# kkrt-labs/stwo-brainfuck

Hardware: AMD Instinct MI355X
Metric: trace cells committed+proved/sec (higher is better)
Workload: dtype u32 (M31 / QM31 modular arithmetic)

## Files before the change

### stwo-brainfuck_amd/csrc/api.hip

```cpp
#include "../../include/bfhip.h"
#include "api_guard.h"
#include <cstdlib>
#include "host/circle.h"
#include "host/quotients.h"
#include "host/hash.h"
#include <cstdio>
#include <vector>
#include <algorithm>
#include <chrono>

using namespace bf;

static thread_local std::string g_err;
void bfhip_set_error(const std::string& s) { g_err = s; }

namespace bf {

void Ctx::ensure_aux() { for (auto& a : aux) if (!a) BF_HIP(hipStreamCreateWithFlags(&a, hipStreamNonBlocking)); }
void Ctx::ensure_side() { if (!stream2) BF_HIP(hipStreamCreateWithFlags(&stream2, hipStreamNonBlocking)); }

void Ctx::init(int dev, u32 max_log_domain, const Ctx* tables_from) {
    int n = 0;
    if (hipGetDeviceCount(&n) != hipSuccess || n == 0) throw HipError("no HIP device: the bfhip backend has no CPU fallback");
    if (dev < 0 || dev >= n) throw HipError("bad device id");
// ... 859 lines not shown
    for (int k = 0; k < N_COMPONENTS; k++) {
        claimed[k] = q_make(claimed_h[k].x, claimed_h[k].y, claimed_h[k].z, claimed_h[k].w);
        total = q_add(total, claimed[k]);
        reports[k] = check_report_init();
    }
    CheckLaunch launches[N_COMPONENTS];
    const CheckLaunch* d_launches = nullptr;
    CheckReportDev* d_reports = nullptr;
    {
        StageBatch sb(c);
        d_reports = c.stage(reports, N_COMPONENTS);
        for (int k = 0; k < N_COMPONENTS; k++) launches[k] = check_launch_of(k, log_sizes[k], rows[k], inter[k], el, claimed[k], d_reports + k);
        d_launches = c.stage(launches, N_COMPONENTS);
        sb.end();
    }
    {
        ProfScope ps(c.stream, "k_check_cells", 0);
        for (int k = 0; k < N_COMPONENTS; k++) check_constraints_launch(c.stream, k, d_launches + k, log_sizes[k]);
    }
    BF_HIP(hipGetLastError());
    c.read_back(reports, d_reports, sizeof reports);
    int32_t n_bad = 0;
    for (int k = 0; k < N_COMPONENTS; k++) { check_report_fill(out[k], reports[k], k, log_sizes[k], claimed[k]); n_bad += reports[k].n_bad_cells != 0; }
    logup_total_h[0] = total.a.a; logup_total_h[1] = total.a.b; logup_total_h[2] = total.b.a; logup_total_h[3] = total.b.b;
    if (n_bad_components) *n_bad_components = n_bad;
    return 0;
    API_CATCH
}
int32_t bfhip_accumulate_quotients(bfhip_ctx* ctx, uint32_t log_size, const uint32_t* const* cols_h, const uint32_t* col_shifts_h, uint32_t n_cols,
                                   const uint32_t* n_samples_h, const uint32_t* sample_points_h, const uint32_t* sample_values_h,
                                   const uint32_t random_coeff_h[4], uint32_t* const out_d[4]) {
    API_CTX(ctx)
    Ctx& c = ctx->c;
    if (log_size < 3 || log_size > c.tw_root_log + 1) throw HipError("accumulate_quotients: log_size outside the twiddle tree");
    std::vector<ColDesc> descs(n_cols);
    std::vector<std::vector<ColumnSample>> samples(n_cols);
    size_t si = 0;
    for (u32 k = 0; k < n_cols; k++) {
        descs[k] = ColDesc{cols_h[k], col_shifts_h ? col_shifts_h[k] : 0u, 0};
        if (descs[k].shift == 1) throw HipError("accumulate_quotients: column shift must be 0 or >= 2");
        for (u32 s = 0; s < n_samples_h[k]; s++, si++) {
            const uint32_t* p = sample_points_h + 8 * si;
            samples[k].push_back({PtQ{q_from_h(p), q_from_h(p + 4)}, q_from_h(sample_values_h + 4 * si)});
        }
    }
    std::vector<QuotientBatch> batches; std::vector<QuotientEntry> entries;
    build_quotient_batches(samples, q_from_h(random_coeff_h), batches, entries);
    quotient_entries_finish(batches.data(), batches.size(), entries.data(), descs.data());
    c.stage_checkpoint();
    QuotientArgs a{};
    a.batches = batches.empty() ? nullptr : c.stage(batches.data(), batches.size());
    a.entries = entries.empty() ? nullptr : c.stage(entries.data(), entries.size());
    a.n_batches = (u32)batches.size(); a.log = log_size; a.tw = c.d_tw; a.tw_total = 1u << c.tw_root_log;
    for (int w = 0; w < 4; w++) a.out[w] = out_d[w];
    const u32 blocks = quotient_groups_layout(&a, 1);
    accumulate_quotients(c.stream, c.stage(&a, 1), 1, blocks);
    BF_HIP(hipGetLastError());
    return 0;
    API_CATCH
}

}

#ifdef BFHIP_TEST_HOOKS
__global__ void __launch_bounds__(256) k_test_field_op(u32 op, const u32* __restrict__ a, const u32* __restrict__ b, u32* __restrict__ out, u32 n) {
    const u32 i = blockIdx.x * blockDim.x + threadIdx.x;
    if (i >= n) return;
    const u32 a0 = a[4 * i], a1 = a[4 * i + 1], a2 = a[4 * i + 2], a3 = a[4 * i + 3];
    const u32 b0 = b[4 * i], b1 = b[4 * i + 1], b2 = b[4 * i + 2], b3 = b[4 * i + 3];
    const u64 a64 = ((u64)a1 << 32) | a0;
    const Q31 x = q_make(a0, a1, a2, a3), y = q_make(b0, b1, b2, b3);
    Q31 r = q_zero();
    switch (op) {
        case 0: r.a.a = m_add(a0, b0); break;
        case 1: r.a.a = m_sub(a0, b0); break;
        case 2: r.a.a = m_mul(a0, b0); break;
        case 3: r.a.a = m_mul_pre2(a0, 2u * b0); break;
        case 4: r.a.a = m_mul_pow2(a0, b0 % 31u); break;
        case 5: r.a.a = m_inv(a0); break;
        case 6: r.a.a = m_red4(a64); break;
        case 7: r.a.a = m_canon(a64); break;
        case 8: r = q_mul(x, y); break;
        case 9: r = q_mul_const(x, q_const(y)); break;
        default: r = q_inv(x); break;
    }
    out[4 * i] = r.a.a; out[4 * i + 1] = r.a.b; out[4 * i + 2] = r.b.a; out[4 * i + 3] = r.b.b;
}
extern "C" int32_t bfhip_test_field_op(bfhip_ctx* ctx, uint32_t op, const uint32_t* a_d, const uint32_t* b_d, uint32_t* out_d, size_t n) {
    API_CTX(ctx)
    if (op > 10) throw HipError("bfhip_test_field_op: unknown op");
    if (!a_d || !b_d || !out_d) throw HipError("null argument");
    if (n == 0 || n > (size_t(1) << 28)) throw HipError("bfhip_test_field_op: n out of range");
    hipLaunchKernelGGL(k_test_field_op, dim3((u32)((n + 255) / 256)), dim3(256), 0, ctx->c.stream, op, a_d, b_d, out_d, (u32)n);
    BF_HIP(hipGetLastError());
    return 0;
    API_CATCH
}
extern "C" int32_t bfhip_test_constraint_group_rows(int32_t component, uint32_t log_size, uint32_t main_shift) {
    if (component < 0 || component >= N_COMPONENTS) { g_err = "unknown component"; return -1; }
    ConstraintLaunch L{};
    for (u32 j = 0; j < n_main_cols(component); j++) L.trace[j].shift = main_shift;
    for (u32 j = 0; j + 4 < 4 * n_logup_cols(component); j++) L.inter[j].shift = main_shift;
    L.log_size = log_size;
    return (int32_t)constraint_group_rows(L, component);
}
#endif
```

### stwo-brainfuck_amd/csrc/kernels.h

```cpp
#pragma once
#include <hip/hip_runtime.h>
#include "m31.h"
#include "air.h"
#include <string>
#include <vector>

struct bfhip_trace;

namespace bf {

struct ColDesc { const u32* ptr; u32 shift; u32 pad_; };

int prof_mode(hipStream_t s);
void prof_enable(hipStream_t s, int mode);
void prof_run_begin(hipStream_t s, const char* name);
void prof_run_end(hipStream_t s);
void prof_begin(hipStream_t s, const char* name, double bytes, double units, double aux = 0.0);
void prof_end(hipStream_t s);
void prof_reset(hipStream_t s);
std::string prof_report_json(const hipStream_t* streams, int n);
void prof_forget(hipStream_t s);
struct ProfScope {
    hipStream_t s; bool on;
    ProfScope(hipStream_t s_, const char* name, double bytes, double units = 0.0, bool dominant = false, double aux = 0.0) : s(s_) {
// ... 54 lines not shown
struct IsFirstCols { u32* ptr[28]; u32 log_min, log_max; };
void is_first_coeffs(hipStream_t stream, const IsFirstCols& a, const u32* itw, u32 tw_root_log);

void merkle_layer(hipStream_t stream, void* out, const void* prev, const ColDesc* d_cols, u32 ncols, u32 log, double col_bytes, u32 out_shift, u32 prev_shift,
                  u32 node_conv, u32 first = 0, u32 count = 0);
struct MerkleTreeDesc { uint4* layers[32]; u32 shifts[32]; u32 col_off[32]; const ColDesc* cols; u32 n_cols, max_log; };
static constexpr u32 MERKLE_SUBTREE_ROOT_LEVEL = 9;
void merkle_subtree(hipStream_t stream, const MerkleTreeDesc& tree, u32 hi, u32 node_conv, double bytes, double compressions);
void merkle_subtree_share(hipStream_t stream, const MerkleTreeDesc& tree, u32 hi, u32 stop, u32 lo, u32 wg0, u32 n_wg, u32 node_conv, double bytes, double compressions);
void merkle_top(hipStream_t stream, const MerkleTreeDesc& tree, u32 top_hi, u32 node_conv, u32* d_chan, u32* d_alpha8, u32* d_root_copy, double bytes, double compressions,
                u32* d_stamp = nullptr, u32 stamp_value = 0);
struct FriTailLayer {
    u32* ev[4];
    const u32* quot[4];
    uint4* tree[11];
};
struct FriTailArgs {
    u32 n_layers, top_log;
    u32 alpha_idx, root_idx;
    u32* ev_last[4];
    u32* chan; u32* alpha; u32* roots;
    const u32* itw; u32 tw_total, rfc;
    FriTailLayer layer[10];
};
void fri_tail(hipStream_t stream, const FriTailArgs* d_args, double bytes, double compressions);
struct FriLayerArgs {
    const u32* src[4]; const u32* quot[4]; u32* dst[4]; uint4* tree[18];
    const u32* alpha8; const u32* itw; u32 tw_total, log, rfc, pad_;
    u32* counter; u32* chan; u32* alpha_out; u32* root_out;
};
void fri_layer(hipStream_t stream, const FriLayerArgs& a);
enum FriFoldMode : int { FF_LINE = 0, FF_LINE_CIRCLE = 1, FF_CIRCLE = 2 };
struct FriFoldLeafArgs { const u32* src[4]; const u32* quot[4]; u32* dst[4]; const u32* alpha8; const u32* itw; u32 tw_total, log; };
void fri_fold_leaf(hipStream_t stream, void* out, const FriFoldLeafArgs& a, int mode, u32 node_conv);
void grind_span(hipStream_t stream, const u32* d_digest, u64 base, u32 span, u32 pow_bits, unsigned long long* d_best, u32 mix_u64_conv);
void clock_probe_launch(hipStream_t stream, uint4* d_stamps, u32* d_sink, u32 blocks, u32 iters);
void clock_sampler_launch(hipStream_t stream, uint4* d_out, const u32* d_stop_alias, unsigned long long max_ticks);
void fill_mix(hipStream_t stream, u32* p, size_t n);
void channel_mix_root_draw(hipStream_t stream, u32* d_chan, const u32* d_root, u32* d_alpha8, u32* d_root_copy);

void merkle_layer_poseidon(hipStream_t stream, void* out, const void* prev, const ColDesc* d_cols, u32 ncols, u32 log, u32 out_shift = 0, u32 prev_shift = 0,
                           u32 first = 0, u32 count = 0);
void hades_once(hipStream_t stream, const u32* d_in24, u32* d_out24);
void grind_poseidon_span(hipStream_t stream, const u32* d_digest, u64 base, u32 span, u32 pow_bits, unsigned long long* d_best);

struct ConstraintLaunch {
    const u32* is_first; ColDesc trace[13]; ColDesc inter[12]; u32* acc[4]; Q31 coeff[12]; Lookups el; Q31 total_sum; u32 denom_inv[2]; u32 log_size;
    u32 overwrite;
    u32 row0, n_rows;
    const u32* inter_prev[4];
};
void eval_constraints(hipStream_t stream, int comp, const ConstraintLaunch* d_args, u32 log_size, u32 n_rows = 0, u32 group_rows = 0);
u32 constraint_group_rows(const ConstraintLaunch& L, int comp);
struct ConstraintClass { u32 n_comps, block0, group_rows, pad_; u32 comp[13]; u32 pad2_[3]; };
struct ConstraintBatch { u32 n_classes, total_blocks, pad_[2]; ConstraintClass cls[13]; };
void constraint_batch_init(ConstraintBatch& b, const ConstraintLaunch* launches, u32 n);
void eval_constraints_batch(hipStream_t stream, const ConstraintBatch* d_batch, const ConstraintBatch& h_batch, const ConstraintLaunch* d_args);
struct LogupLaunch {
    const u32* cols[13];
    u32* out_rep[8];
    u32* out_last[4];
    void* vrow; void* wloc; void* totals; void* claimed;
    Lookups el; u32 log_rows; int comp;
};
struct LogupItem { const u32* cols[13]; u32* out_rep[8]; u32* out_last[4]; uint4* vrow; uint4* wloc; uint4* totals; uint4* claimed; u32 log_rows; int comp; u32 nb; u32 pad_; };
struct LogupBatch { Lookups el; u32 n; u32 rows_blk0[14], scan_blk0[14], last_blk0[14]; u32 pad_; LogupItem item[13]; };
void logup_batch_init(LogupBatch& b, const Lookups& el, const LogupLaunch* L, u32 n);
void logup_batch_run(hipStream_t stream, const LogupBatch* d_batch, const LogupBatch& h_batch);
void broadcast16(hipStream_t stream, const u32* d_rows, u32* d_out, u32 n_cells);

struct CheckReportDev { u64 n_bad_cells, first_bad_cell; u64 bad_per_constraint[16]; u32 first_bad_constraint; u32 first_bad_value[4]; u32 pad_[3]; };
struct CheckLaunch { ColDesc trace[13]; ColDesc inter[12]; Lookups el; Q31 total_sum; u32 log_size; u32 pad_; CheckReportDev* report; };
void check_constraints_launch(hipStream_t stream, int comp, const CheckLaunch* d_args, u32 log_size);

void trace_columns(const bfhip_trace* t, const u32* cols[N_COMPONENTS][13], u32 log_sizes[N_COMPONENTS]);

const u32* exclusive_scan_u32(hipStream_t s, const u32* in, u32* out, u32* totals, u32 n);

struct EvalJob { const u32* coeffs; u32 log_n; u32 point; u32 factor_shift; u32 partial_off; u32 out_idx; u32 pad_; };
void eval_at_points(hipStream_t stream, const EvalJob* d_jobs, u32 n_jobs, u32 total_partials, const void* d_factors, void* d_partials, void* d_out);
struct QuotientBatch { C31 prx, pry, pix, piy; Q31 a_sum, b_sum, batch_coeff; u32 n_cols; C31 kden; u32 n_full; };
struct QuotientEntry { Q31 c; const u32* ptr; u32 shift; u32 col; };
void quotient_entries_finish(QuotientBatch* batches, size_t n_batches, QuotientEntry* entries, const ColDesc* cols);
struct QuotientArgs { const QuotientBatch* batches; const QuotientEntry* entries; u32 n_batches; u32 log; const u32* tw; u32 tw_total; u32* out[4]; u32 row0, n_rows; u32 block0, pad_; };
u32 quotient_groups_layout(QuotientArgs* h_groups, u32 n_groups);
void accumulate_quotients(hipStream_t stream, const QuotientArgs* d_groups, u32 n_groups, u32 total_blocks);
void fold_circle_into_line(hipStream_t stream, u32* const dst[4], const u32* const src[4], const u32* d_alpha8, const u32* itw, u32 tw_root_log, u32 log, bool fresh = false,
                           u32 first = 0, u32 count = 0);
void fold_line(hipStream_t stream, u32* const dst[4], const u32* const src[4], const u32* d_alpha8, const u32* itw, u32 tw_root_log, u32 log, u32 first = 0, u32 count = 0);
void fold_line_circle(hipStream_t stream, u32* const dst[4], const u32* const src[4], const u32* const quot[4], const u32* d_alpha8, const u32* itw, u32 tw_root_log, u32 log,
                      u32 first = 0, u32 count = 0);
void prev_row_copy(hipStream_t stream, u32* dst, const u32* src, u32 log_size);
struct GatherReq { const u32* base; u64 index; u32 out_off; u32 n_words; };
void gather_u32(hipStream_t stream, const GatherReq* d_req, u32 n, u32* d_out);
void accumulate(hipStream_t stream, u32* dst, const u32* src, u32 n);
struct AccumulateSizes { u32* dst[4]; const u32* src[12][4]; u32 log[12]; u32 n; };
void accumulate_sizes(hipStream_t stream, const AccumulateSizes& a);
void batch_inverse_m31(hipStream_t stream, const u32* src, u32* dst, u32 n);
void batch_inverse_qm31(hipStream_t stream, const u32* const src[4], u32* const dst[4], u32 n);
void bit_reverse(hipStream_t stream, const u32* src, u32* dst, u32 log);
void one_hot(hipStream_t stream, u32* dst, u32 n);

struct TraceSoA { const u32 *clk, *ip, *ci, *ni, *mp, *mv, *mvi; u32 n; };
struct Ctx;
TraceSoA ingest_registers(Ctx& c, const u32* trace7_h, size_t n_rows, u64* first_bad);

}
```

### stwo-brainfuck_amd/csrc/m31.h

```cpp
#pragma once
#include <cstdint>
#include <cstddef>

#if defined(__HIPCC__)
#include <hip/hip_runtime.h>
#define BF_HD __host__ __device__ __forceinline__
#else
#define BF_HD inline
#endif

namespace bf {

using u8 = uint8_t;
using u32 = uint32_t;
using u64 = uint64_t;

constexpr u32 P31 = 0x7fffffffu;

struct Conventions {
    u32 merkle_node_hash = 0;
    u32 mix_u64 = 0;
    u32 logup_mask_order = 0;
    u32 merkle_channel = 0;
};

struct PcsConfig {
    u32 pow_bits = 5, log_blowup = 1, log_last_layer_degree_bound = 0, n_queries = 3;
    bool is_default() const { return pow_bits == 5 && log_blowup == 1 && log_last_layer_degree_bound == 0 && n_queries == 3; }
};

BF_HD u32 m_add(u32 a, u32 b) { u32 s = a + b; u32 t = s - P31; return t < s ? t : s; }
BF_HD u32 m_sub(u32 a, u32 b) { u32 s = a - b; u32 t = s + P31; return t < s ? t : s; }
BF_HD u64 m_fold(u64 x) { return (x & P31) + (x >> 31); }
BF_HD u32 m_canon(u64 x) { x = m_fold(m_fold(x)); u32 r = (u32)x; return r >= P31 ? r - P31 : r; }
BF_HD u32 m_neg(u32 a) { return a ? P31 - a : 0; }
BF_HD u32 m_reduce64(u64 x) {
    u32 lo = (u32)x & P31, hi = (u32)(x >> 31);
    u32 s = lo + hi; u32 t = s - P31; return t < s ? t : s;
}
BF_HD u32 m_mul(u32 a, u32 b) { return m_reduce64((u64)a * b); }
BF_HD u32 m_mul_pre2(u32 a, u32 w2) {
    u64 p = (u64)a * w2;
    u32 s = (u32)(p >> 32) + ((u32)p >> 1); u32 t = s - P31; return t < s ? t : s;
}
BF_HD u32 m_mul_pow2(u32 a, u32 k) { return ((a << k) & P31) | (a >> (31u - k)); }
BF_HD u32 m_sqr(u32 a) { return m_mul(a, a); }
BF_HD u32 m_inv_pow2(u32 n) { return 1u << ((31u - n % 31u) % 31u); }
BF_HD u32 m_pow(u32 b, u32 e) { u32 r = 1; while (e) { if (e & 1) r = m_mul(r, b); b = m_mul(b, b); e >>= 1; } return r; }
BF_HD u32 m_sqn(u32 x, int n) { for (int i = 0; i < n; i++) x = m_sqr(x); return x; }
BF_HD u32 m_inv(u32 x) {
    u32 t0 = m_mul(m_sqn(x, 2), x);
    u32 t1 = m_mul(m_sqr(t0), t0);
    u32 t2 = m_mul(m_sqn(t1, 3), t0);
    u32 t3 = m_mul(m_sqr(t2), t0);
    u32 t4 = m_mul(m_sqn(t3, 8), t3);
    u32 t5 = m_mul(m_sqn(t4, 8), t3);
    return m_mul(m_sqn(t5, 7), t2);
}

struct C31 { u32 a, b; };
BF_HD C31 c_add(C31 x, C31 y) { return {m_add(x.a, y.a), m_add(x.b, y.b)}; }
BF_HD C31 c_sub(C31 x, C31 y) { return {m_sub(x.a, y.a), m_sub(x.b, y.b)}; }
BF_HD C31 c_neg(C31 x) { return {m_neg(x.a), m_neg(x.b)}; }
BF_HD C31 c_mul(C31 x, C31 y) { return {m_sub(m_mul(x.a, y.a), m_mul(x.b, y.b)), m_add(m_mul(x.a, y.b), m_mul(x.b, y.a))}; }
BF_HD C31 c_mulm(C31 x, u32 y) { return {m_mul(x.a, y), m_mul(x.b, y)}; }
BF_HD C31 c_mulR(C31 x) { return {m_sub(m_add(x.a, x.a), x.b), m_add(x.a, m_add(x.b, x.b))}; }
BF_HD C31 c_inv(C31 x) { u32 n = m_inv(m_add(m_sqr(x.a), m_sqr(x.b))); return {m_mul(x.a, n), m_neg(m_mul(x.b, n))}; }

struct Q31 { C31 a, b; };
BF_HD Q31 q_make(u32 a0, u32 a1, u32 a2, u32 a3) { return {{a0, a1}, {a2, a3}}; }
BF_HD Q31 q_zero() { return {{0, 0}, {0, 0}}; }
BF_HD Q31 q_one() { return {{1, 0}, {0, 0}}; }
BF_HD Q31 q_from_m(u32 x) { return {{x, 0}, {0, 0}}; }
BF_HD Q31 q_add(Q31 x, Q31 y) { return {c_add(x.a, y.a), c_add(x.b, y.b)}; }
BF_HD Q31 q_sub(Q31 x, Q31 y) { return {c_sub(x.a, y.a), c_sub(x.b, y.b)}; }
BF_HD Q31 q_neg(Q31 x) { return {c_neg(x.a), c_neg(x.b)}; }
BF_HD Q31 q_mul(Q31 x, Q31 y) { return {c_add(c_mul(x.a, y.a), c_mulR(c_mul(x.b, y.b))), c_add(c_mul(x.a, y.b), c_mul(x.b, y.a))}; }
BF_HD Q31 q_mulm(Q31 x, u32 y) { return {c_mulm(x.a, y), c_mulm(x.b, y)}; }
struct QConst { u32 c0, c1, c2, c3, e0, e1, nc1, nc3, ne1; };
BF_HD QConst q_const(Q31 y) {
    const C31 e = c_mulR(y.b);
    return {y.a.a, y.a.b, y.b.a, y.b.b, e.a, e.b, P31 - y.a.b, P31 - y.b.b, P31 - e.b};
}
BF_HD u32 m_red4(u64 x) {
    const u64 t = ((x >> 32) << 1) + (u32)x;
    const u32 s = ((u32)t & P31) + (u32)(t >> 31); const u32 d = s - P31; return d < s ? d : s;
}
BF_HD Q31 q_mul_const(Q31 x, const QConst& k) {
    const u64 a0 = x.a.a, a1 = x.a.b, b0 = x.b.a, b1 = x.b.b;
    return q_make(m_red4(a0 * k.c0 + a1 * k.nc1 + b0 * k.e0 + b1 * k.ne1), m_red4(a0 * k.c1 + a1 * k.c0 + b0 * k.e1 + b1 * k.e0),
                  m_red4(a0 * k.c2 + a1 * k.nc3 + b0 * k.c0 + b1 * k.nc1), m_red4(a0 * k.c3 + a1 * k.c2 + b0 * k.c1 + b1 * k.c0));
}
BF_HD Q31 q_mulc(Q31 x, C31 y) { return {c_mul(x.a, y), c_mul(x.b, y)}; }
BF_HD Q31 q_addm(Q31 x, u32 y) { x.a.a = m_add(x.a.a, y); return x; }
BF_HD Q31 q_subm(Q31 x, u32 y) { x.a.a = m_sub(x.a.a, y); return x; }
BF_HD Q31 q_conj(Q31 x) { return {x.a, c_neg(x.b)}; }
BF_HD Q31 q_inv(Q31 x) { C31 d = c_inv(c_sub(c_mul(x.a, x.a), c_mulR(c_mul(x.b, x.b)))); return {c_mul(x.a, d), c_neg(c_mul(x.b, d))}; }
BF_HD bool q_eq(Q31 x, Q31 y) { return x.a.a == y.a.a && x.a.b == y.a.b && x.b.a == y.b.a && x.b.b == y.b.b; }
BF_HD bool q_is_zero(Q31 x) { return (x.a.a | x.a.b | x.b.a | x.b.b) == 0; }
BF_HD Q31 q_pow(Q31 b, u64 e) { Q31 r = q_one(); while (e) { if (e & 1) r = q_mul(r, b); b = q_mul(b, b); e >>= 1; } return r; }

BF_HD u32 bit_rev(u32 i, u32 log) {
#if defined(__HIP_DEVICE_COMPILE__)
    return log ? (__brev(i) >> (32 - log)) : 0;
#else
    u32 r = 0; for (u32 k = 0; k < log; k++) r |= ((i >> k) & 1u) << (log - 1 - k); return r;
#endif
}

}
```

### stwo-brainfuck_amd/csrc/quotient.hip

```cpp
#include <algorithm>
#include "kernels.h"
#include <stdexcept>

namespace bf {

__device__ __forceinline__ Q31 ld_q(const uint4* p, size_t i) { uint4 v = p[i]; return q_make(v.x, v.y, v.z, v.w); }
__device__ __forceinline__ uint4 pk_q(Q31 q) { return make_uint4(q.a.a, q.a.b, q.b.a, q.b.b); }

static constexpr u32 EAP_CHUNK_LOG = 12;

__global__ void __launch_bounds__(256) k_eval_at_point_stage1(const EvalJob* __restrict__ jobs, u32 n_jobs, const uint4* __restrict__ factors, uint4* __restrict__ partials) {
    u32 lo_j = 0, hi_j = n_jobs;
    while (hi_j - lo_j > 1) { u32 mid = (lo_j + hi_j) >> 1; if (jobs[mid].partial_off <= blockIdx.x) lo_j = mid; else hi_j = mid; }
    const EvalJob job = jobs[lo_j];
    const u32 n = 1u << job.log_n;
    const u32 chunk = blockIdx.x - job.partial_off;
    __shared__ uint4 s_w[16];
    __shared__ uint4 s_p[256];
    const uint4* F = factors + (size_t)job.point * 32 + job.factor_shift;
    const u32 t = threadIdx.x;
    if (t < 16) {
        Q31 w = q_one();
        for (u32 b = 0; b < 4; b++) if ((t >> b) & 1) w = q_mul(w, ld_q(F, b));
        s_w[t] = pk_q(w);
// ... 8 lines not shown
#pragma unroll
            for (u32 v4 = 0; v4 < 4; v4++) {
                const uint4 c = src[v4];
                const u32 cv[4] = {c.x, c.y, c.z, c.w};
#pragma unroll
                for (u32 j = 0; j < 4; j++) {
                    const u32 idx = v4 * 4 + j;
                    if (idx % 4 == 0 && idx) { a64[0] = m_fold(a64[0]); a64[1] = m_fold(a64[1]); a64[2] = m_fold(a64[2]); a64[3] = m_fold(a64[3]); }
                    const Q31 w = ld_q(s_w, idx);
                    a64[0] += (u64)w.a.a * cv[j]; a64[1] += (u64)w.a.b * cv[j]; a64[2] += (u64)w.b.a * cv[j]; a64[3] += (u64)w.b.b * cv[j];
                }
            }
            acc = q_make(m_red4(a64[0]), m_red4(a64[1]), m_red4(a64[2]), m_red4(a64[3]));
        } else {
            for (u32 k = 0; k < n; k++) acc = q_add(acc, q_mulm(ld_q(s_w, k), job.coeffs[k]));
        }
    }
    s_p[t] = pk_q(acc);
    __syncthreads();
    for (u32 b = 0; b < 8; b++) {
        u32 half = 128u >> b;
        Q31 r;
        bool act = t < half;
        if (act) {
            Q31 lo = ld_q(s_p, 2 * t), hi = ld_q(s_p, 2 * t + 1);
            r = (4 + b < job.log_n) ? q_add(lo, q_mul_const(hi, q_const(ld_q(F, 4 + b)))) : lo;
        }
        __syncthreads();
        if (act) s_p[t] = pk_q(r);
        __syncthreads();
    }
    if (t == 0) partials[(size_t)job.partial_off + chunk] = s_p[0];
}

__global__ void __launch_bounds__(256) k_eval_at_point_stage2(const EvalJob* __restrict__ jobs, const uint4* __restrict__ factors, const uint4* __restrict__ partials, uint4* __restrict__ out) {
    const EvalJob job = jobs[blockIdx.x];
    const u32 nchunks = job.log_n > EAP_CHUNK_LOG ? 1u << (job.log_n - EAP_CHUNK_LOG) : 1u;
    const uint4* F = factors + (size_t)job.point * 32 + job.factor_shift;
    const uint4* p = partials + job.partial_off;
    __shared__ uint4 s[256];
    const u32 t = threadIdx.x;
    u32 lanes = nchunks < 256 ? nchunks : 256;
    u32 per_log = 0; while ((lanes << per_log) < nchunks) per_log++;
    Q31 acc = q_zero();
    if (t < lanes) {
        u32 per = 1u << per_log;
        for (u32 k = 0; k < per; k++) {
            Q31 w = q_one();
            for (u32 b = 0; b < per_log; b++) if ((k >> b) & 1) w = q_mul(w, ld_q(F, EAP_CHUNK_LOG + b));
            acc = q_add(acc, q_mul(ld_q(p, ((size_t)t << per_log) + k), w));
        }
    }
    s[t] = pk_q(acc);
    __syncthreads();
    u32 lanes_log = 0; while ((1u << lanes_log) < lanes) lanes_log++;
    for (u32 b = 0; b < lanes_log; b++) {
        u32 half = lanes >> (b + 1);
        Q31 r; bool act = t < half;
        if (act) r = q_add(ld_q(s, 2 * t), q_mul_const(ld_q(s, 2 * t + 1), q_const(ld_q(F, EAP_CHUNK_LOG + per_log + b))));
        __syncthreads();
        if (act) s[t] = pk_q(r);
        __syncthreads();
    }
    if (t == 0) out[job.out_idx] = s[0];
}

void eval_at_points(hipStream_t stream, const EvalJob* d_jobs, u32 n_jobs, u32 total_partials, const void* d_factors, void* d_partials, void* d_out) {
    if (!n_jobs) return;
    hipLaunchKernelGGL(k_eval_at_point_stage1, dim3(total_partials), dim3(256), 0, stream, d_jobs, n_jobs, (const uint4*)d_factors, (uint4*)d_partials);
    hipLaunchKernelGGL(k_eval_at_point_stage2, dim3(n_jobs), dim3(256), 0, stream, d_jobs, (const uint4*)d_factors, (const uint4*)d_partials, (uint4*)d_out);
}

__device__ __forceinline__ void domain_point(const u32* __restrict__ tw, u32 tw_total, u32 log, u32 row, u32& x, u32& y) {
    const u32* t1 = tw + (tw_total - (1u << (log - 1)));
    u32 xv = t1[row >> 2];
    x = (row & 2) ? m_neg(xv) : xv;
    u32 h = row >> 1;
    u32 cx = t1[(h >> 2) * 2], cy = t1[(h >> 2) * 2 + 1];
    u32 sel = h & 3;
    u32 yv = sel == 0 ? cy : sel == 1 ? m_neg(cy) : sel == 2 ? m_neg(cx) : cx;
    y = (row & 1) ? m_neg(yv) : yv;
}

__global__ void __launch_bounds__(256) k_quotients(const QuotientArgs* __restrict__ groups, u32 n_groups) {
    u32 g = 0;
    while (g + 1 < n_groups && groups[g + 1].block0 <= blockIdx.x) g++;
    const QuotientArgs& a = groups[g];
    u32 row0 = ((blockIdx.x - a.block0) * blockDim.x + threadIdx.x) * 4;
    if (a.n_rows) { if (row0 >= a.n_rows) return; row0 += a.row0; }
    else if (row0 >= (1u << a.log)) return;
    u32 xv, yv;
    domain_point(a.tw, a.tw_total, a.log, row0, xv, yv);
    Q31 acc[4] = {q_zero(), q_zero(), q_zero(), q_zero()};
    u32 e = 0;
    for (u32 b = 0; b < a.n_batches; b++) {
        const QuotientBatch qb = ld_constant(a.batches + b);
        u64 n64[4][4], s64[4];
#pragma unroll
        for (int r = 0; r < 4; r++) { n64[r][0] = 0; n64[r][1] = 0; n64[r][2] = 0; n64[r][3] = 0; }
        s64[0] = 0; s64[1] = 0; s64[2] = 0; s64[3] = 0;
        const QuotientEntry* ent = a.entries + e;
        e += qb.n_cols;
        const u32 nf = qb.n_full, nr = qb.n_cols - qb.n_full;
        if (nf) {
            uint4 A[3], B[3];
            const u32 last = nf - 1;
            auto load3 = [&](uint4 (&buf)[3], u32 k) {
#pragma unroll
                for (u32 j = 0; j < 3; j++) buf[j] = ld16(as_global(ld_constant(&ent[min(k + j, last)].ptr)) + row0);
            };
            auto mac3 = [&](const uint4 (&buf)[3], u32 k) {
#pragma unroll
                for (int r = 0; r < 4; r++) { n64[r][0] = m_fold(n64[r][0]); n64[r][1] = m_fold(n64[r][1]); n64[r][2] = m_fold(n64[r][2]); n64[r][3] = m_fold(n64[r][3]); }
#pragma unroll
                for (u32 j = 0; j < 3; j++) {
                    if (k + j < nf) {
                        const Q31 cc = ld_constant(&ent[k + j].c);
                        const u32 vr[4] = {buf[j].x, buf[j].y, buf[j].z, buf[j].w};
#pragma unroll
                        for (int r = 0; r < 4; r++) { n64[r][0] += (u64)cc.a.a * vr[r]; n64[r][1] += (u64)cc.a.b * vr[r]; n64[r][2] += (u64)cc.b.a * vr[r]; n64[r][3] += (u64)cc.b.b * vr[r]; }
                    }
                }
            };
            load3(A, 0);
            for (u32 k = 0; k < nf; k += 6) {
                load3(B, k + 3);
                mac3(A, k);
                load3(A, k + 6);
                mac3(B, k + 3);
            }
        }
        if (nr) {
            const QuotientEntry* er = ent + nf;
            u32 A[3], B[3];
            const u32 last = nr - 1;
            auto load3 = [&](u32 (&buf)[3], u32 k) {
#pragma unroll
                for (u32 j = 0; j < 3; j++) { const u32 i = min(k + j, last); buf[j] = as_global(ld_constant(&er[i].ptr))[row0 >> ld_constant(&er[i].shift)]; }
            };
            auto mac3 = [&](const u32 (&buf)[3], u32 k) {
                s64[0] = m_fold(s64[0]); s64[1] = m_fold(s64[1]); s64[2] = m_fold(s64[2]); s64[3] = m_fold(s64[3]);
#pragma unroll
                for (u32 j = 0; j < 3; j++) {
                    if (k + j < nr) {
                        const Q31 cc = ld_constant(&er[k + j].c);
                        s64[0] += (u64)cc.a.a * buf[j]; s64[1] += (u64)cc.a.b * buf[j]; s64[2] += (u64)cc.b.a * buf[j]; s64[3] += (u64)cc.b.b * buf[j];
                    }
                }
            };
            load3(A, 0);
            for (u32 k = 0; k < nr; k += 6) {
                load3(B, k + 3);
                mac3(A, k);
                load3(A, k + 6);
                mac3(B, k + 3);
            }
        }
        const Q31 ay = q_mulm(qb.a_sum, yv);
        const Q31 line_p = q_add(qb.b_sum, ay), line_m = q_sub(qb.b_sum, ay);
        const C31 P = {m_mul(xv, qb.piy.a), m_mul(xv, qb.piy.b)}, Q = {m_mul(yv, qb.pix.a), m_mul(yv, qb.pix.b)};
        const C31 km = c_sub(qb.kden, P), kp = c_add(qb.kden, P);
        C31 den[4] = {c_add(km, Q), c_sub(km, Q), c_sub(kp, Q), c_add(kp, Q)};
        Q31 num[4]; u32 nrm[4];
#pragma unroll
        for (int r = 0; r < 4; r++) {
            num[r] = q_make(m_canon(m_fold(n64[r][0]) + m_fold(s64[0])), m_canon(m_fold(n64[r][1]) + m_fold(s64[1])),
                            m_canon(m_fold(n64[r][2]) + m_fold(s64[2])), m_canon(m_fold(n64[r][3]) + m_fold(s64[3])));
            num[r] = q_sub(num[r], (r == 0 || r == 3) ? line_p : line_m);
            nrm[r] = m_add(m_sqr(den[r].a), m_sqr(den[r].b));
        }
        u32 p01 = m_mul(nrm[0], nrm[1]), p012 = m_mul(p01, nrm[2]), inv_all = m_inv(m_mul(p012, nrm[3]));
        u32 i3 = m_mul(inv_all, p012), t3 = m_mul(inv_all, nrm[3]);
        u32 i2 = m_mul(t3, p01), t2 = m_mul(t3, nrm[2]);
        u32 i1 = m_mul(t2, nrm[0]), i0 = m_mul(t2, nrm[1]);
        u32 ninv[4] = {i0, i1, i2, i3};
#pragma unroll
        for (int r = 0; r < 4; r++) {
            C31 dinv = {m_mul(den[r].a, ninv[r]), m_neg(m_mul(den[r].b, ninv[r]))};
            Q31 term = q_mulc(num[r], dinv);
            acc[r] = b ? q_add(acc[r], term) : term;
        }
    }
    *reinterpret_cast<uint4*>(a.out[0] + row0) = make_uint4(acc[0].a.a, acc[1].a.a, acc[2].a.a, acc[3].a.a);
    *reinterpret_cast<uint4*>(a.out[1] + row0) = make_uint4(acc[0].a.b, acc[1].a.b, acc[2].a.b, acc[3].a.b);
    *reinterpret_cast<uint4*>(a.out[2] + row0) = make_uint4(acc[0].b.a, acc[1].b.a, acc[2].b.a, acc[3].b.a);
    *reinterpret_cast<uint4*>(a.out[3] + row0) = make_uint4(acc[0].b.b, acc[1].b.b, acc[2].b.b, acc[3].b.b);
}
void quotient_entries_finish(QuotientBatch* batches, size_t n_batches, QuotientEntry* entries, const ColDesc* cols) {
    for (size_t b = 0; b < n_batches; b++) {
        QuotientEntry* first = entries; QuotientEntry* last = entries + batches[b].n_cols;
        for (QuotientEntry* q = first; q != last; q++) { q->ptr = cols[q->col].ptr; q->shift = cols[q->col].shift; }
        batches[b].n_full = (u32)(std::stable_partition(first, last, [](const QuotientEntry& q) { return q.shift == 0; }) - first);
        entries = last;
    }
}
u32 quotient_groups_layout(QuotientArgs* h_groups, u32 n_groups) {
    u32 blocks = 0;
    for (u32 g = 0; g < n_groups; g++) {
        const u32 lanes = (h_groups[g].n_rows ? h_groups[g].n_rows : (1u << h_groups[g].log)) / 4;
        h_groups[g].block0 = blocks;
        blocks += (lanes + 255) / 256;
    }
    return blocks;
}
void accumulate_quotients(hipStream_t stream, const QuotientArgs* d_groups, u32 n_groups, u32 total_blocks) {
    if (!n_groups || !total_blocks) return;
    ProfScope ps(stream, "k_quotients", 0);
    hipLaunchKernelGGL(k_quotients, dim3(total_blocks), dim3(256), 0, stream, d_groups, n_groups);
}

__global__ void __launch_bounds__(256) k_fold_circle_into_line(u32* const d0, u32* const d1, u32* const d2, u32* const d3,
                                                               const u32* __restrict__ s0, const u32* __restrict__ s1, const u32* __restrict__ s2, const u32* __restrict__ s3,
                                                               const u32* __restrict__ alpha8, const u32* __restrict__ itw, u32 tw_total, u32 log, u32 fresh, u32 first, u32 count) {
    u32 i = blockIdx.x * blockDim.x + threadIdx.x;
    if (i >= count) return;
    i += first;
    const QConst alpha = q_const(q_make(alpha8[0], alpha8[1], alpha8[2], alpha8[3])), alpha_sq = q_const(q_make(alpha8[4], alpha8[5], alpha8[6], alpha8[7]));
    const u32* t1 = itw + (tw_total - (1u << (log - 1)));
    u32 cx = t1[(i >> 2) * 2], cy = t1[(i >> 2) * 2 + 1], sel = i & 3;
    u32 yinv = sel == 0 ? cy : sel == 1 ? m_neg(cy) : sel == 2 ? m_neg(cx) : cx;
    uint2 a0 = reinterpret_cast<const uint2*>(s0)[i], a1 = reinterpret_cast<const uint2*>(s1)[i], a2 = reinterpret_cast<const uint2*>(s2)[i], a3 = reinterpret_cast<const uint2*>(s3)[i];
    Q31 fp = q_make(a0.x, a1.x, a2.x, a3.x), fn = q_make(a0.y, a1.y, a2.y, a3.y);
    Q31 f0 = q_add(fp, fn), f1 = q_mulm(q_sub(fp, fn), yinv);
    Q31 fprime = q_add(q_mul_const(f1, alpha), f0);
    Q31 r = fprime;
    if (!fresh) { Q31 dst = q_make(d0[i], d1[i], d2[i], d3[i]); r = q_add(q_mul_const(dst, alpha_sq), fprime); }
    d0[i] = r.a.a; d1[i] = r.a.b; d2[i] = r.b.a; d3[i] = r.b.b;
}
__global__ void __launch_bounds__(256) k_fold_line(u32* __restrict__ d0, u32* __restrict__ d1, u32* __restrict__ d2, u32* __restrict__ d3,
                                                   const u32* __restrict__ s0, const u32* __restrict__ s1, const u32* __restrict__ s2, const u32* __restrict__ s3,
                                                   const u32* __restrict__ alpha8, const u32* __restrict__ itw, u32 tw_total, u32 log, u32 first, u32 count) {
    u32 i = blockIdx.x * blockDim.x + threadIdx.x;
    if (i >= count) return;
    i += first;
    const QConst alpha = q_const(q_make(alpha8[0], alpha8[1], alpha8[2], alpha8[3]));
    u32 xinv = itw[tw_total - (1u << log) + i];
    uint2 a0 = reinterpret_cast<const uint2*>(s0)[i], a1 = reinterpret_cast<const uint2*>(s1)[i], a2 = reinterpret_cast<const uint2*>(s2)[i], a3 = reinterpret_cast<const uint2*>(s3)[i];
    Q31 fx = q_make(a0.x, a1.x, a2.x, a3.x), fn = q_make(a0.y, a1.y, a2.y, a3.y);
    Q31 f0 = q_add(fx, fn), f1 = q_mulm(q_sub(fx, fn), xinv);
    Q31 r = q_add(f0, q_mul_const(f1, alpha));
    d0[i] = r.a.a; d1[i] = r.a.b; d2[i] = r.b.a; d3[i] = r.b.b;
}
__global__ void __launch_bounds__(256) k_fold_line_circle(u32* __restrict__ d0, u32* __restrict__ d1, u32* __restrict__ d2, u32* __restrict__ d3,
                                                          const u32* __restrict__ s0, const u32* __restrict__ s1, const u32* __restrict__ s2, const u32* __restrict__ s3,
                                                          const u32* __restrict__ q0, const u32* __restrict__ q1, const u32* __restrict__ q2, const u32* __restrict__ q3,
                                                          const u32* __restrict__ alpha8, const u32* __restrict__ itw, u32 tw_total, u32 log, u32 first, u32 count) {
    u32 i = blockIdx.x * blockDim.x + threadIdx.x;
    if (i >= count) return;
    i += first;
    const QConst alpha = q_const(q_make(alpha8[0], alpha8[1], alpha8[2], alpha8[3]));
    Q31 r;
    {
        const u32 xinv = itw[tw_total - (1u << log) + i];
        const uint2 a0 = reinterpret_cast<const uint2*>(s0)[i], a1 = reinterpret_cast<const uint2*>(s1)[i], a2 = reinterpret_cast<const uint2*>(s2)[i], a3 = reinterpret_cast<const uint2*>(s3)[i];
        const Q31 fx = q_make(a0.x, a1.x, a2.x, a3.x), fn = q_make(a0.y, a1.y, a2.y, a3.y);
        r = q_add(q_add(fx, fn), q_mul_const(q_mulm(q_sub(fx, fn), xinv), alpha));
    }
    if (q0) {
        const QConst alpha_sq = q_const(q_make(alpha8[4], alpha8[5], alpha8[6], alpha8[7]));
        const u32* t1 = itw + (tw_total - (1u << (log - 1)));
        const u32 cx = t1[(i >> 2) * 2], cy = t1[(i >> 2) * 2 + 1], sel = i & 3;
        const u32 yinv = sel == 0 ? cy : sel == 1 ? m_neg(cy) : sel == 2 ? m_neg(cx) : cx;
        const uint2 a0 = reinterpret_cast<const uint2*>(q0)[i], a1 = reinterpret_cast<const uint2*>(q1)[i], a2 = reinterpret_cast<const uint2*>(q2)[i], a3 = reinterpret_cast<const uint2*>(q3)[i];
        const Q31 fp = q_make(a0.x, a1.x, a2.x, a3.x), fn = q_make(a0.y, a1.y, a2.y, a3.y);
        const Q31 fprime = q_add(q_mul_const(q_mulm(q_sub(fp, fn), yinv), alpha), q_add(fp, fn));
        r = q_add(q_mul_const(r, alpha_sq), fprime);
    }
    d0[i] = r.a.a; d1[i] = r.a.b; d2[i] = r.b.a; d3[i] = r.b.b;
}
void fold_line_circle(hipStream_t stream, u32* const dst[4], const u32* const src[4], const u32* const quot[4], const u32* d_alpha8, const u32* itw, u32 tw_root_log, u32 log,
                      u32 first, u32 count) {
    if (!count) { first = 0; count = 1u << (log - 1); }
    hipLaunchKernelGGL(k_fold_line_circle, dim3((count + 255) / 256), dim3(256), 0, stream, dst[0], dst[1], dst[2], dst[3], src[0], src[1], src[2], src[3],
                       quot ? quot[0] : nullptr, quot ? quot[1] : nullptr, quot ? quot[2] : nullptr, quot ? quot[3] : nullptr, d_alpha8, itw, 1u << tw_root_log, log, first, count);
}

void fold_circle_into_line(hipStream_t stream, u32* const dst[4], const u32* const src[4], const u32* d_alpha8, const u32* itw, u32 tw_root_log, u32 log, bool fresh,
                           u32 first, u32 count) {
    if (!count) { first = 0; count = 1u << (log - 1); }
    hipLaunchKernelGGL(k_fold_circle_into_line, dim3((count + 255) / 256), dim3(256), 0, stream, dst[0], dst[1], dst[2], dst[3], src[0], src[1], src[2], src[3],
                       d_alpha8, itw, 1u << tw_root_log, log, fresh ? 1u : 0u, first, count);
}
// ... 101 lines not shown
```

Before: 14.37 billion.

## Batch quotient denominator inversions across four batches and widen single-batch lanes

Restructures the quotient kernel so each lane computes denominators for up to four batches (or four quads of rows in the single-batch case), stores them in shared memory, and shares one field inversion across all of them (Montgomery batch inversion). When a group has a single batch, each lane handles 16 rows and writes terms directly, so one inversion covers sixteen rows. The column loads use a deeper 4-entry prefetch pipeline, and a lazy complex multiply skips some reductions. This trades inversion cost for 32KB of shared memory per block, which may reduce occupancy, and for added code complexity.

```diff
diff --git a/stwo-brainfuck_amd/csrc/api.hip b/stwo-brainfuck_amd/csrc/api.hip
--- a/stwo-brainfuck_amd/csrc/api.hip
+++ b/stwo-brainfuck_amd/csrc/api.hip
@@ -965,19 +965,27 @@
         case 7: r.a.a = m_canon(a64); break;
         case 8: r = q_mul(x, y); break;
         case 9: r = q_mul_const(x, q_const(y)); break;
-        default: r = q_inv(x); break;
+        case 10: r = q_inv(x); break;
+        case 11: r.a.a = c_norm(x.a); break;
+        default: r = q_mulc_lazy(x, y.a); break;
     }
     out[4 * i] = r.a.a; out[4 * i + 1] = r.a.b; out[4 * i + 2] = r.b.a; out[4 * i + 3] = r.b.b;
 }
 extern "C" int32_t bfhip_test_field_op(bfhip_ctx* ctx, uint32_t op, const uint32_t* a_d, const uint32_t* b_d, uint32_t* out_d, size_t n) {
     API_CTX(ctx)
-    if (op > 10) throw HipError("bfhip_test_field_op: unknown op");
+    if (op > 12) throw HipError("bfhip_test_field_op: unknown op");
     if (!a_d || !b_d || !out_d) throw HipError("null argument");
     if (n == 0 || n > (size_t(1) << 28)) throw HipError("bfhip_test_field_op: n out of range");
     hipLaunchKernelGGL(k_test_field_op, dim3((u32)((n + 255) / 256)), dim3(256), 0, ctx->c.stream, op, a_d, b_d, out_d, (u32)n);
     BF_HIP(hipGetLastError());
     return 0;
     API_CATCH
+}
+extern "C" int32_t bfhip_test_quotient_rows_per_lane(uint32_t log_size, uint32_t n_rows, uint32_t n_batches) {
+    QuotientArgs a{};
+    a.log = log_size; a.n_rows = n_rows; a.n_batches = n_batches;
+    quotient_groups_layout(&a, 1);
+    return (int32_t)a.rows_per_lane;
 }
 extern "C" int32_t bfhip_test_constraint_group_rows(int32_t component, uint32_t log_size, uint32_t main_shift) {
     if (component < 0 || component >= N_COMPONENTS) { g_err = "unknown component"; return -1; }
diff --git a/stwo-brainfuck_amd/csrc/kernels.h b/stwo-brainfuck_amd/csrc/kernels.h
--- a/stwo-brainfuck_amd/csrc/kernels.h
+++ b/stwo-brainfuck_amd/csrc/kernels.h
@@ -160,7 +160,7 @@
 struct QuotientBatch { C31 prx, pry, pix, piy; Q31 a_sum, b_sum, batch_coeff; u32 n_cols; C31 kden; u32 n_full; };
 struct QuotientEntry { Q31 c; const u32* ptr; u32 shift; u32 col; };
 void quotient_entries_finish(QuotientBatch* batches, size_t n_batches, QuotientEntry* entries, const ColDesc* cols);
-struct QuotientArgs { const QuotientBatch* batches; const QuotientEntry* entries; u32 n_batches; u32 log; const u32* tw; u32 tw_total; u32* out[4]; u32 row0, n_rows; u32 block0, pad_; };
+struct QuotientArgs { const QuotientBatch* batches; const QuotientEntry* entries; u32 n_batches; u32 log; const u32* tw; u32 tw_total; u32* out[4]; u32 row0, n_rows; u32 block0, rows_per_lane; };
 u32 quotient_groups_layout(QuotientArgs* h_groups, u32 n_groups);
 void accumulate_quotients(hipStream_t stream, const QuotientArgs* d_groups, u32 n_groups, u32 total_blocks);
 void fold_circle_into_line(hipStream_t stream, u32* const dst[4], const u32* const src[4], const u32* d_alpha8, const u32* itw, u32 tw_root_log, u32 log, bool fresh = false,
diff --git a/stwo-brainfuck_amd/csrc/m31.h b/stwo-brainfuck_amd/csrc/m31.h
--- a/stwo-brainfuck_amd/csrc/m31.h
+++ b/stwo-brainfuck_amd/csrc/m31.h
@@ -92,6 +92,12 @@
                   m_red4(a0 * k.c2 + a1 * k.nc3 + b0 * k.c0 + b1 * k.nc1), m_red4(a0 * k.c3 + a1 * k.c2 + b0 * k.c1 + b1 * k.c0));
 }
 BF_HD Q31 q_mulc(Q31 x, C31 y) { return {c_mul(x.a, y), c_mul(x.b, y)}; }
+BF_HD u32 c_norm(C31 x) { return m_red4((u64)x.a * x.a + (u64)x.b * x.b); }
+BF_HD C31 c_mul_lazy(C31 x, C31 y) {
+    const u32 nb = P31 - y.b;
+    return {m_red4((u64)x.a * y.a + (u64)x.b * nb), m_red4((u64)x.a * y.b + (u64)x.b * y.a)};
+}
+BF_HD Q31 q_mulc_lazy(Q31 x, C31 y) { return {c_mul_lazy(x.a, y), c_mul_lazy(x.b, y)}; }
 BF_HD Q31 q_addm(Q31 x, u32 y) { x.a.a = m_add(x.a.a, y); return x; }
 BF_HD Q31 q_subm(Q31 x, u32 y) { x.a.a = m_sub(x.a.a, y); return x; }
 BF_HD Q31 q_conj(Q31 x) { return {x.a, c_neg(x.b)}; }
diff --git a/stwo-brainfuck_amd/csrc/quotient.hip b/stwo-brainfuck_amd/csrc/quotient.hip
--- a/stwo-brainfuck_amd/csrc/quotient.hip
+++ b/stwo-brainfuck_amd/csrc/quotient.hip
@@ -114,109 +114,164 @@
     y = (row & 1) ? m_neg(yv) : yv;
 }
 
+
+__device__ __forceinline__ void quad_dens(const QuotientBatch& qb, u32 xv, u32 yv, C31 (&den)[4]) {
+    const C31 P = {m_mul(xv, qb.piy.a), m_mul(xv, qb.piy.b)}, Q = {m_mul(yv, qb.pix.a), m_mul(yv, qb.pix.b)};
+    const C31 km = c_sub(qb.kden, P), kp = c_add(qb.kden, P);
+    den[0] = c_add(km, Q); den[1] = c_sub(km, Q); den[2] = c_sub(kp, Q); den[3] = c_add(kp, Q);
+}
+
+template <bool SETTLE> __device__ __forceinline__ void quad_numerators(const QuotientEntry* ent, u32 nf, u32 nr, u32 row0, Q31 (&num)[4]) {
+    u64 n64[4][4], s64[4];
+#pragma unroll
+    for (int r = 0; r < 4; r++) { n64[r][0] = 0; n64[r][1] = 0; n64[r][2] = 0; n64[r][3] = 0; }
+    s64[0] = 0; s64[1] = 0; s64[2] = 0; s64[3] = 0;
+    if (nf) {
+        uint4 buf[4];
+        const u32 last = nf - 1;
+        auto load = [&](u32 k) { return ld16(as_global(ld_constant(&ent[min(k, last)].ptr)) + row0); };
+#pragma unroll
+        for (u32 j = 0; j < 4; j++) buf[j] = load(j);
+        if (SETTLE) __builtin_amdgcn_s_waitcnt(0x0F70);
+        for (u32 k = 0; k < nf; k += 4) {
+#pragma unroll
+            for (int r = 0; k && r < 4; r++) { n64[r][0] = m_fold(n64[r][0]); n64[r][1] = m_fold(n64[r][1]); n64[r][2] = m_fold(n64[r][2]); n64[r][3] = m_fold(n64[r][3]); }
+#pragma unroll
+            for (u32 j = 0; j < 4; j++) {
+                if (k + j < nf) {
+                    const Q31 cc = ld_constant(&ent[k + j].c);
+                    const u32 vr[4] = {buf[j].x, buf[j].y, buf[j].z, buf[j].w};
+#pragma unroll
+                    for (int r = 0; r < 4; r++) { n64[r][0] += (u64)cc.a.a * vr[r]; n64[r][1] += (u64)cc.a.b * vr[r]; n64[r][2] += (u64)cc.b.a * vr[r]; n64[r][3] += (u64)cc.b.b * vr[r]; }
+                }
+                buf[j] = load(k + 4 + j);
+            }
+        }
+    }
+    if (nr) {
+        const QuotientEntry* er = ent + nf;
+        u32 buf[4];
+        const u32 last = nr - 1;
+        auto load = [&](u32 k) { const u32 i = min(k, last); return as_global(ld_constant(&er[i].ptr))[row0 >> ld_constant(&er[i].shift)]; };
+#pragma unroll
+        for (u32 j = 0; j < 4; j++) buf[j] = load(j);
+        if (SETTLE && !nf) __builtin_amdgcn_s_waitcnt(0x0F70);
+        for (u32 k = 0; k < nr; k += 4) {
+            if (k) { s64[0] = m_fold(s64[0]); s64[1] = m_fold(s64[1]); s64[2] = m_fold(s64[2]); s64[3] = m_fold(s64[3]); }
+#pragma unroll
+            for (u32 j = 0; j < 4; j++) {
+                if (k + j < nr) {
+                    const Q31 cc = ld_constant(&er[k + j].c);
+                    s64[0] += (u64)cc.a.a * buf[j]; s64[1] += (u64)cc.a.b * buf[j]; s64[2] += (u64)cc.b.a * buf[j]; s64[3] += (u64)cc.b.b * buf[j];
+                }
+                buf[j] = load(k + 4 + j);
+            }
+        }
+    }
+    const u64 sf[4] = {m_fold(s64[0]), m_fold(s64[1]), m_fold(s64[2]), m_fold(s64[3])};
+#pragma unroll
+    for (int r = 0; r < 4; r++) num[r] = q_make(m_reduce64(m_fold(n64[r][0]) + sf[0]), m_reduce64(m_fold(n64[r][1]) + sf[1]), m_reduce64(m_fold(n64[r][2]) + sf[2]), m_reduce64(m_fold(n64[r][3]) + sf[3]));
+}
+
+template <bool WIDE> __device__ __forceinline__ void quotients_lane(const QuotientArgs& a, u32 lane, u32 lanes, u32 base, u32 (*s_dinv)[256]) {
+    const u32 t = threadIdx.x;
+    auto quad_row = [&](u32 g) { return base + ((WIDE ? g * lanes : 0u) + lane) * 4; };
+    u32 xv0 = 0, yv0 = 0;
+    if (!WIDE) domain_point(a.tw, a.tw_total, a.log, quad_row(0), xv0, yv0);
+    Q31 acc[4] = {q_zero(), q_zero(), q_zero(), q_zero()};
+    u32 e = 0;
+    const u32 n_batches = WIDE ? 1u : a.n_batches;
+    for (u32 b0 = 0; b0 < n_batches; b0 += 4) {
+        const u32 cnt = WIDE ? 4u : min(4u, n_batches - b0);
+        {
+            u32 nrm[4][4], PG[4], G[4], run = 1;
+#pragma unroll
+            for (u32 g = 0; g < 4; g++) {
+                if (g < cnt) {
+                    const QuotientBatch* pb = a.batches + (WIDE ? 0u : b0 + g);
+                    QuotientBatch qb;
+                    qb.pix = ld_constant(&pb->pix); qb.piy = ld_constant(&pb->piy); qb.kden = ld_constant(&pb->kden);
+                    u32 xv = xv0, yv = yv0;
+                    if (WIDE) domain_point(a.tw, a.tw_total, a.log, quad_row(g), xv, yv);
+                    C31 den[4];
+                    quad_dens(qb, xv, yv, den);
+#pragma unroll
+                    for (int r = 0; r < 4; r++) { s_dinv[2 * (4 * g + r)][t] = den[r].a; s_dinv[2 * (4 * g + r) + 1][t] = den[r].b; nrm[g][r] = c_norm(den[r]); }
+                    G[g] = m_mul(m_mul(m_mul(nrm[g][0], nrm[g][1]), nrm[g][2]), nrm[g][3]);
+                    PG[g] = run; run = g ? m_mul(run, G[g]) : G[g];
+                }
+            }
+            u32 inv = m_inv(run);
+#pragma unroll
+            for (int g = 3; g >= 0; g--) {
+                if ((u32)g < cnt) {
+                    const u32 i_pair = g ? m_mul(inv, PG[g]) : inv;
+                    if (g) inv = m_mul(inv, G[g]);
+                    const u32 p01 = m_mul(nrm[g][0], nrm[g][1]), p012 = m_mul(p01, nrm[g][2]);
+                    const u32 i3 = m_mul(i_pair, p012), t3 = m_mul(i_pair, nrm[g][3]);
+                    const u32 i2 = m_mul(t3, p01), t2 = m_mul(t3, nrm[g][2]);
+                    const u32 ninv[4] = {m_mul(t2, nrm[g][1]), m_mul(t2, nrm[g][0]), i2, i3};
+#pragma unroll
+                    for (int r = 0; r < 4; r++) {
+                        const C31 den = {s_dinv[2 * (4 * g + r)][t], s_dinv[2 * (4 * g + r) + 1][t]};
+                        s_dinv[2 * (4 * g + r)][t] = m_mul(den.a, ninv[r]); s_dinv[2 * (4 * g + r) + 1][t] = m_neg(m_mul(den.b, ninv[r]));
+                    }
+                }
+            }
+        }
+        for (u32 g = 0; g < cnt; g++) {
+            const QuotientBatch qb = ld_constant(a.batches + (WIDE ? 0u : b0 + g));
+            const u32 row0 = quad_row(g);
+            const QuotientEntry* ent = a.entries + e;
+            if (!WIDE) e += qb.n_cols;
+            u32 xv = xv0, yv = yv0;
+            if (WIDE) domain_point(a.tw, a.tw_total, a.log, row0, xv, yv);
+            Q31 num[4];
+            quad_numerators<WIDE>(ent, qb.n_full, qb.n_cols - qb.n_full, row0, num);
+            const Q31 ay = q_mulm(qb.a_sum, yv);
+            const Q31 line_p = q_add(qb.b_sum, ay), line_m = q_sub(qb.b_sum, ay);
+            Q31 term[4];
+#pragma unroll
+            for (int r = 0; r < 4; r++) {
+                const C31 dinv = {s_dinv[2 * (4 * g + r)][t], s_dinv[2 * (4 * g + r) + 1][t]};
+                term[r] = q_mulc_lazy(q_sub(num[r], (r == 0 || r == 3) ? line_p : line_m), dinv);
+            }
+            if (WIDE) {
+                *reinterpret_cast<uint4*>(a.out[0] + row0) = make_uint4(term[0].a.a, term[1].a.a, term[2].a.a, term[3].a.a);
+                *reinterpret_cast<uint4*>(a.out[1] + row0) = make_uint4(term[0].a.b, term[1].a.b, term[2].a.b, term[3].a.b);
+                *reinterpret_cast<uint4*>(a.out[2] + row0) = make_uint4(term[0].b.a, term[1].b.a, term[2].b.a, term[3].b.a);
+                *reinterpret_cast<uint4*>(a.out[3] + row0) = make_uint4(term[0].b.b, term[1].b.b, term[2].b.b, term[3].b.b);
+            } else {
+#pragma unroll
+                for (int r = 0; r < 4; r++) acc[r] = (b0 + g) ? q_add(acc[r], term[r]) : term[r];
+            }
+        }
+    }
+    if (!WIDE) {
+        const u32 row0 = quad_row(0);
+        *reinterpret_cast<uint4*>(a.out[0] + row0) = make_uint4(acc[0].a.a, acc[1].a.a, acc[2].a.a, acc[3].a.a);
+        *reinterpret_cast<uint4*>(a.out[1] + row0) = make_uint4(acc[0].a.b, acc[1].a.b, acc[2].a.b, acc[3].a.b);
+        *reinterpret_cast<uint4*>(a.out[2] + row0) = make_uint4(acc[0].b.a, acc[1].b.a, acc[2].b.a, acc[3].b.a);
+        *reinterpret_cast<uint4*>(a.out[3] + row0) = make_uint4(acc[0].b.b, acc[1].b.b, acc[2].b.b, acc[3].b.b);
+    }
+}
+
 __global__ void __launch_bounds__(256) k_quotients(const QuotientArgs* __restrict__ groups, u32 n_groups) {
+    __shared__ u32 s_dinv[32][256];
     u32 g = 0;
     while (g + 1 < n_groups && groups[g + 1].block0 <= blockIdx.x) g++;
     const QuotientArgs& a = groups[g];
-    u32 row0 = ((blockIdx.x - a.block0) * blockDim.x + threadIdx.x) * 4;
-    if (a.n_rows) { if (row0 >= a.n_rows) return; row0 += a.row0; }
-    else if (row0 >= (1u << a.log)) return;
-    u32 xv, yv;
-    domain_point(a.tw, a.tw_total, a.log, row0, xv, yv);
-    Q31 acc[4] = {q_zero(), q_zero(), q_zero(), q_zero()};
-    u32 e = 0;
-    for (u32 b = 0; b < a.n_batches; b++) {
-        const QuotientBatch qb = ld_constant(a.batches + b);
-        u64 n64[4][4], s64[4];
-#pragma unroll
-        for (int r = 0; r < 4; r++) { n64[r][0] = 0; n64[r][1] = 0; n64[r][2] = 0; n64[r][3] = 0; }
-        s64[0] = 0; s64[1] = 0; s64[2] = 0; s64[3] = 0;
-        const QuotientEntry* ent = a.entries + e;
-        e += qb.n_cols;
-        const u32 nf = qb.n_full, nr = qb.n_cols - qb.n_full;
-        if (nf) {
-            uint4 A[3], B[3];
-            const u32 last = nf - 1;
-            auto load3 = [&](uint4 (&buf)[3], u32 k) {
-#pragma unroll
-                for (u32 j = 0; j < 3; j++) buf[j] = ld16(as_global(ld_constant(&ent[min(k + j, last)].ptr)) + row0);
-            };
-            auto mac3 = [&](const uint4 (&buf)[3], u32 k) {
-#pragma unroll
-                for (int r = 0; r < 4; r++) { n64[r][0] = m_fold(n64[r][0]); n64[r][1] = m_fold(n64[r][1]); n64[r][2] = m_fold(n64[r][2]); n64[r][3] = m_fold(n64[r][3]); }
-#pragma unroll
-                for (u32 j = 0; j < 3; j++) {
-                    if (k + j < nf) {
-                        const Q31 cc = ld_constant(&ent[k + j].c);
-                        const u32 vr[4] = {buf[j].x, buf[j].y, buf[j].z, buf[j].w};
-#pragma unroll
-                        for (int r = 0; r < 4; r++) { n64[r][0] += (u64)cc.a.a * vr[r]; n64[r][1] += (u64)cc.a.b * vr[r]; n64[r][2] += (u64)cc.b.a * vr[r]; n64[r][3] += (u64)cc.b.b * vr[r]; }
-                    }
-                }
-            };
-            load3(A, 0);
-            for (u32 k = 0; k < nf; k += 6) {
-                load3(B, k + 3);
-                mac3(A, k);
-                load3(A, k + 6);
-                mac3(B, k + 3);
-            }
-        }
-        if (nr) {
-            const QuotientEntry* er = ent + nf;
-            u32 A[3], B[3];
-            const u32 last = nr - 1;
-            auto load3 = [&](u32 (&buf)[3], u32 k) {
-#pragma unroll
-                for (u32 j = 0; j < 3; j++) { const u32 i = min(k + j, last); buf[j] = as_global(ld_constant(&er[i].ptr))[row0 >> ld_constant(&er[i].shift)]; }
-            };
-            auto mac3 = [&](const u32 (&buf)[3], u32 k) {
-                s64[0] = m_fold(s64[0]); s64[1] = m_fold(s64[1]); s64[2] = m_fold(s64[2]); s64[3] = m_fold(s64[3]);
-#pragma unroll
-                for (u32 j = 0; j < 3; j++) {
-                    if (k + j < nr) {
-                        const Q31 cc = ld_constant(&er[k + j].c);
-                        s64[0] += (u64)cc.a.a * buf[j]; s64[1] += (u64)cc.a.b * buf[j]; s64[2] += (u64)cc.b.a * buf[j]; s64[3] += (u64)cc.b.b * buf[j];
-                    }
-                }
-            };
-            load3(A, 0);
-            for (u32 k = 0; k < nr; k += 6) {
-                load3(B, k + 3);
-                mac3(A, k);
-                load3(A, k + 6);
-                mac3(B, k + 3);
-            }
-        }
-        const Q31 ay = q_mulm(qb.a_sum, yv);
-        const Q31 line_p = q_add(qb.b_sum, ay), line_m = q_sub(qb.b_sum, ay);
-        const C31 P = {m_mul(xv, qb.piy.a), m_mul(xv, qb.piy.b)}, Q = {m_mul(yv, qb.pix.a), m_mul(yv, qb.pix.b)};
-        const C31 km = c_sub(qb.kden, P), kp = c_add(qb.kden, P);
-        C31 den[4] = {c_add(km, Q), c_sub(km, Q), c_sub(kp, Q), c_add(kp, Q)};
-        Q31 num[4]; u32 nrm[4];
-#pragma unroll
-        for (int r = 0; r < 4; r++) {
-            num[r] = q_make(m_canon(m_fold(n64[r][0]) + m_fold(s64[0])), m_canon(m_fold(n64[r][1]) + m_fold(s64[1])),
-                            m_canon(m_fold(n64[r][2]) + m_fold(s64[2])), m_canon(m_fold(n64[r][3]) + m_fold(s64[3])));
-            num[r] = q_sub(num[r], (r == 0 || r == 3) ? line_p : line_m);
-            nrm[r] = m_add(m_sqr(den[r].a), m_sqr(den[r].b));
-        }
-        u32 p01 = m_mul(nrm[0], nrm[1]), p012 = m_mul(p01, nrm[2]), inv_all = m_inv(m_mul(p012, nrm[3]));
-        u32 i3 = m_mul(inv_all, p012), t3 = m_mul(inv_all, nrm[3]);
-        u32 i2 = m_mul(t3, p01), t2 = m_mul(t3, nrm[2]);
-        u32 i1 = m_mul(t2, nrm[0]), i0 = m_mul(t2, nrm[1]);
-        u32 ninv[4] = {i0, i1, i2, i3};
-#pragma unroll
-        for (int r = 0; r < 4; r++) {
-            C31 dinv = {m_mul(den[r].a, ninv[r]), m_neg(m_mul(den[r].b, ninv[r]))};
-            Q31 term = q_mulc(num[r], dinv);
-            acc[r] = b ? q_add(acc[r], term) : term;
-        }
-    }
-    *reinterpret_cast<uint4*>(a.out[0] + row0) = make_uint4(acc[0].a.a, acc[1].a.a, acc[2].a.a, acc[3].a.a);
-    *reinterpret_cast<uint4*>(a.out[1] + row0) = make_uint4(acc[0].a.b, acc[1].a.b, acc[2].a.b, acc[3].a.b);
-    *reinterpret_cast<uint4*>(a.out[2] + row0) = make_uint4(acc[0].b.a, acc[1].b.a, acc[2].b.a, acc[3].b.a);
-    *reinterpret_cast<uint4*>(a.out[3] + row0) = make_uint4(acc[0].b.b, acc[1].b.b, acc[2].b.b, acc[3].b.b);
+    const u32 lane = (blockIdx.x - a.block0) * blockDim.x + threadIdx.x;
+    const u32 rows = a.n_rows ? a.n_rows : (1u << a.log);
+    const u32 lanes = rows / a.rows_per_lane;
+    if (lane >= lanes) return;
+    const u32 base = a.n_rows ? a.row0 : 0u;
+#ifdef BF_QUOT_ONLY_ROWS
+    quotients_lane<BF_QUOT_ONLY_ROWS == 16>(a, lane, lanes, base, s_dinv);
+#else
+    if (a.rows_per_lane == 16) quotients_lane<true>(a, lane, lanes, base, s_dinv);
+    else quotients_lane<false>(a, lane, lanes, base, s_dinv);
+#endif
 }
 void quotient_entries_finish(QuotientBatch* batches, size_t n_batches, QuotientEntry* entries, const ColDesc* cols) {
     for (size_t b = 0; b < n_batches; b++) {
@@ -229,7 +284,9 @@
 u32 quotient_groups_layout(QuotientArgs* h_groups, u32 n_groups) {
     u32 blocks = 0;
     for (u32 g = 0; g < n_groups; g++) {
-        const u32 lanes = (h_groups[g].n_rows ? h_groups[g].n_rows : (1u << h_groups[g].log)) / 4;
+        const u32 rows = h_groups[g].n_rows ? h_groups[g].n_rows : (1u << h_groups[g].log);
+        h_groups[g].rows_per_lane = (h_groups[g].n_batches == 1 && rows % 16 == 0) ? 16u : 4u;
+        const u32 lanes = rows / h_groups[g].rows_per_lane;
         h_groups[g].block0 = blocks;
         blocks += (lanes + 255) / 256;
     }
```

After: 14.39 billion (median of 2 runs). About the same (+0.1%).
